# AppleHolic/pytorch_sound

Hardware: AMD Instinct MI355X
Metric: audio-sec/s STFT+mel+fwd/bwd (higher is better)
Workload: dtype bf16; 1 GPU; configs[1]: Conv1d separator (4 x ResBlock1, C=256, on 513-bin magnitude), 22.05 kHz, STFT 1024/256, 80 mel, batch 32 x 2 s per GPU, Adam, bf16 autocast; global_batch=32, parallelism=dp1, model_params=5520386

## Files before the change

pytorch_sound_amd/csrc/psnd_conv.hip:

```cpp
#include "psnd_common.h"
#include "psnd_conv_pair.h"
#include <stdlib.h>
#include <string.h>
#include <algorithm>
#include <atomic>

namespace {

typedef __attribute__((ext_vector_type(8))) short bf16x8;
typedef __attribute__((ext_vector_type(16))) float f32x16;
typedef unsigned short bf16_t;

__device__ __forceinline__ float bf2f(bf16_t v) { return __builtin_bit_cast(float, (unsigned)v << 16); }
__device__ __forceinline__ bf16_t f2bf(float f) {
    unsigned u = __builtin_bit_cast(unsigned, f);
    if ((u & 0x7fffffffu) > 0x7f800000u) return (bf16_t)((u >> 16) | 0x40);
    u += 0x7fffu + ((u >> 16) & 1u);
    return (bf16_t)(u >> 16);
}

typedef __bf16 hwbf16x2 __attribute__((ext_vector_type(2)));
typedef float f32x2_t __attribute__((ext_vector_type(2)));
__device__ __forceinline__ unsigned pack_bf16(float lo, float hi) {
    const f32x2_t v = {lo, hi};
// ... 446 lines not shown
    float l1acc = 0.f;
#pragma unroll
    for (int i = 0; i < 4; ++i) {
        const int j = ty + 8 * i, c = c0 + j, t = t0 + tx;
        if (c < C && t < T) {
            const size_t o = clip + (size_t)c * T + t;
            const float v = MASK ? tile[tx][j] * m[i] : tile[tx][j];
            out[o] = v;
            if (l1) l1acc += fabsf(v - r[i]);
        }
    }
    if (MASK && l1_part) {
        double d = (double)l1acc;
#pragma unroll
        for (int m = 32; m >= 1; m >>= 1) d += __shfl_xor(d, m, 64);
        __shared__ double red[4];
        if ((threadIdx.x & 63) == 0) red[threadIdx.x >> 6] = d;
        __syncthreads();
        if (threadIdx.x == 0)
            l1_part[((size_t)blockIdx.z * gridDim.y + blockIdx.y) * gridDim.x + blockIdx.x] = red[0] + red[1] + red[2] + red[3];
    }
}

constexpr int WKT = 3;
struct WgradParams {
    const bf16_t *G1, *G2, *GM;
    const bf16_t *xa;
    float *gw, *gbias;
    bf16_t *g_out;
    long long R;
    int Ca, Cb, k, off0, dstep, rows_per_split;
    float g2_slope;
    int up_u, up_p, up_Lp, up_HP, up_LpO, up_HPO, up_Cr;
#ifdef PSND_TRACE
    long long *trace;
#endif
};
#ifdef PSND_TRACE
#define PSND_WSTAMP(i_)                                                                                         \
    do {                                                                                                        \
        if ((threadIdx.x & 63) == 0 && p.trace)                                                                 \
            p.trace[(tblk * 4 + (threadIdx.x >> 6)) * 8 + (i_)] = __builtin_amdgcn_s_memtime(); \
    } while (0)
#else
#define PSND_WSTAMP(i_)
#endif

#ifndef PSND_WD
#define PSND_WD 2
#endif
constexpr int WD = PSND_WD;
#ifndef PSND_WGRAD_WAVES
#define PSND_WGRAD_WAVES 2
#endif
constexpr int kWgradLdsBytes = 2 * (1 + WKT) * 64 * RS * (int)sizeof(bf16_t);
__device__ __forceinline__ void conv_wgrad_body_v1(const WgradParams &p, const int bx, const int by, const int bz, bf16_t *sT, const size_t tblk) {
    const int tid = threadIdx.x, wave = tid >> 6, lane = tid & 63;
    const int wm = wave >> 1, wn = wave & 1, li = lane & 31, kg = lane >> 5;
    const int co0 = bx * 64, ci0 = by * 64;
    const int ntg = (p.k + WKT - 1) / WKT;
    const int split = bz / ntg, tgrp = bz - split * ntg;
    const long long rs = (long long)split * p.rows_per_split;
    const long long re = min(rs + p.rows_per_split, p.R);
    const int rr = tid & 31, cg = tid >> 5;
    const bool do_bias = (by == 0) && tgrp == 0;
    const bool comb = p.G2 != nullptr;
// ... 124 lines not shown
                    }
                }
        }
    }
    PSND_WSTAMP(3);
#ifdef PSND_TRACE
    __builtin_amdgcn_s_waitcnt(0);
    PSND_WSTAMP(4);
#endif
    if (do_bias && p.gbias) {
#pragma unroll
        for (int e = 0; e < 8; ++e) {
            float v = bsum[e];
#pragma unroll
            for (int m = 16; m >= 1; m >>= 1) v += __shfl_xor(v, m, 64);
            if (rr == 0 && co0 + 8 * cg + e < p.Cb) p.gbias[(size_t)split * p.Cb + co0 + 8 * cg + e] = v;
        }
    }
}
typedef short v4s_t __attribute__((ext_vector_type(4)));
#ifndef PSND_WGRAD_TR
#define PSND_WGRAD_TR 1
#endif
constexpr int WTP = 96;
constexpr int WXR = 64;
static_assert(2 * (32 + WXR) * WTP * (int)sizeof(bf16_t) <= kWgradLdsBytes, "the transposing-read tiles fit version 1's LDS");
__device__ __forceinline__ bf16x8 tr_frag(const bf16_t *p0) {
    const v4s_t a = __builtin_amdgcn_ds_read_tr16_b64_v4i16((v4s_t __attribute__((address_space(3))) *)(p0));
    const v4s_t b = __builtin_amdgcn_ds_read_tr16_b64_v4i16((v4s_t __attribute__((address_space(3))) *)(p0 + 4 * WTP));
    return __builtin_shufflevector(a, b, 0, 1, 2, 3, 4, 5, 6, 7);
}
constexpr int WXRN = 96;
constexpr int kWgradNarrowLdsBytes = 2 * (32 + WXRN) * WTP * (int)sizeof(bf16_t);
template <bool COMB, bool NARROW = false, int WK = WKT>
__device__ __forceinline__ void conv_wgrad_body(const WgradParams &p, const int bx, const int by, const int bz, bf16_t *sT, const size_t tblk) {
#if !PSND_WGRAD_TR
    conv_wgrad_body_v1(p, bx, by, bz, sT, tblk);
#else
    constexpr int XU = NARROW ? 3 : 2, XR = NARROW ? WXRN : WXR, TPW = NARROW ? 4 * WK : WK;
    const int tid = threadIdx.x, wave = tid >> 6, lane = tid & 63;
    const int wm = NARROW ? 0 : wave >> 1, wn = NARROW ? 0 : wave & 1, li = lane & 31, kg = lane >> 5;
    const int co0 = bx * 64, ci0 = by * 64;
    const int ntg = (p.k + TPW - 1) / TPW;
    const int split = bz / ntg, tgrp = bz - split * ntg;
    const long long rs = (long long)split * p.rows_per_split;
    const long long re = min(rs + p.rows_per_split, p.R);
    const int rr = tid >> 3, cg = tid & 7;
    const bool do_bias = (by == 0) && tgrp == 0;
    constexpr bool comb = COMB;
    const bool gok = co0 + 8 * cg < p.Cb, xok = ci0 + 8 * cg < p.Ca;
    float bsum[8] = {0.f, 0.f, 0.f, 0.f, 0.f, 0.f, 0.f, 0.f};
    PSND_WSTAMP(0);
    constexpr unsigned OOB = 0xffffffffu;
    const int g_bytes = (int)((size_t)p.R * p.Cb * sizeof(bf16_t));
    const int x_bytes = p.up_u > 0 ? (int)((size_t)(p.R / p.up_Lp) * p.up_LpO * p.up_Cr * sizeof(bf16_t)) : (int)((size_t)p.R * p.Ca * sizeof(bf16_t));
    const bool haveG1 = p.G1 != nullptr;
    const __amdgpu_buffer_rsrc_t rG1 = make_uniform_rsrc(haveG1 ? p.G1 : p.G2, g_bytes);
    const __amdgpu_buffer_rsrc_t rG2 = make_uniform_rsrc(comb ? p.G2 : p.G1, g_bytes);
    const __amdgpu_buffer_rsrc_t rGM = make_uniform_rsrc(comb ? p.GM : p.G1, g_bytes);
    const __amdgpu_buffer_rsrc_t rX = make_uniform_rsrc(p.xa, x_bytes);
    auto ld16 = [&](__amdgpu_buffer_rsrc_t r, unsigned off) __attribute__((always_inline)) {
        const auto v = __builtin_amdgcn_raw_buffer_load_b128(r, (int)off, 0, 0);
        return __builtin_bit_cast(uint4, v);
    };
    const int tw0 = tgrp * TPW, ntw = min(TPW, p.k - tw0);
    const int t0 = NARROW ? tw0 + wave * WK : tw0;
    const int nt = max(0, min(WK, p.k - t0));
// ... 35 lines not shown
            vx[s][u] = ld16(rX, ok ? (unsigned)((xo + ci0 + 8 * cg) * sizeof(bf16_t)) : OOB);
        }
    };
    auto stage = [&](auto sc, long long r0, bf16_t *sG, bf16_t *sX) __attribute__((always_inline)) {
        constexpr int s = decltype(sc)::value;
        uint4 g = vg[s];
        if constexpr (COMB) {
            const unsigned *pv = reinterpret_cast<const unsigned *>(&vg[s]), *pg = reinterpret_cast<const unsigned *>(&vg2[s]),
                           *pm = reinterpret_cast<const unsigned *>(&vgm[s]);
            unsigned out[4];
#pragma unroll
            for (int i = 0; i < 4; ++i) {
                const float a0 = bf2f((bf16_t)(pv[i] & 0xffff)), a1 = bf2f((bf16_t)(pv[i] >> 16));
                const float b0 = bf2f((bf16_t)(pg[i] & 0xffff)), b1 = bf2f((bf16_t)(pg[i] >> 16));
                const float m0 = bf2f((bf16_t)(pm[i] & 0xffff)), m1 = bf2f((bf16_t)(pm[i] >> 16));
                out[i] = pack_bf16(a0 + b0 * (m0 > 0.f ? 1.f : p.g2_slope), a1 + b1 * (m1 > 0.f ? 1.f : p.g2_slope));
            }
            g = make_uint4(out[0], out[1], out[2], out[3]);
        }
        if (do_bias) {
            const unsigned *pg4 = reinterpret_cast<const unsigned *>(&g);
#pragma unroll
            for (int e = 0; e < 8; ++e) bsum[e] += bf2f((bf16_t)((pg4[e >> 1] >> (16 * (e & 1))) & 0xffff));
            const long long r = r0 + rr;
            if (p.g_out && r < re && gok) *reinterpret_cast<uint4 *>(p.g_out + (size_t)r * p.Cb + co0 + 8 * cg) = g;
        }
        *reinterpret_cast<uint4 *>(sG + rr * WTP + 8 * cg) = g;
        *reinterpret_cast<uint4 *>(sX + rr * WTP + 8 * cg) = vx[s][0];
        if (rr + 32 < xrows) *reinterpret_cast<uint4 *>(sX + (rr + 32) * WTP + 8 * cg) = vx[s][1];
        if constexpr (NARROW)
            if (rr + 64 < xrows) *reinterpret_cast<uint4 *>(sX + (rr + 64) * WTP + 8 * cg) = vx[s][2];
    };
    const int trow = 8 * kg + ((lane & 15) >> 2), tcol = 16 * ((lane >> 4) & 1) + 4 * (lane & 3);
    const int nchunk = ((int)((re - rs + 31) / 32) + WD - 1) / WD * WD;
    static_for<0, WD>([&](auto sc) __attribute__((always_inline)) { fetch(sc, rs + 32ll * decltype(sc)::value); });
    for (int c = 0; c < nchunk; c += WD) {
        static_for<0, WD>([&](auto sc) __attribute__((always_inline)) {
            constexpr int s = decltype(sc)::value;
            const int ch = c + s;
            bf16_t *sG = sT + (ch & 1) * (32 + XR) * WTP, *sX = sG + 32 * WTP;
            if (ch == 4) PSND_WSTAMP(5);
            stage(sc, rs + 32ll * ch, sG, sX);
            if (ch == 0) PSND_WSTAMP(1);
            if (ch == 4) PSND_WSTAMP(6);
            __syncthreads();
            if (ch == 4) PSND_WSTAMP(7);
            fetch(sc, rs + 32ll * (ch + WD));
            bf16x8 fa[2], fb[2][WK];
#pragma unroll
            for (int kk = 0; kk < 2; ++kk) {
                fa[kk] = tr_frag(sG + (16 * kk + trow) * WTP + wm * 32 + tcol);
#pragma unroll
                for (int j = 0; j < WK; ++j) fb[kk][j] = tr_frag(sX + (16 * kk + trow + toff[j]) * WTP + wn * 32 + tcol);
            }
#pragma unroll
            for (int kk = 0; kk < 2; ++kk)
#pragma unroll
                for (int j = 0; j < WK; ++j) acc[j] = __builtin_amdgcn_mfma_f32_32x32x16_bf16(fa[kk], fb[kk][j], acc[j], 0, 0, 0);
        });
    }
    __syncthreads();
    PSND_WSTAMP(2);
    if constexpr (NARROW) {
        constexpr int EPN = 36;
        float *sE = reinterpret_cast<float *>(sT);
        static_assert(4 * 32 * EPN * 4 <= kWgradNarrowLdsBytes, "four 32 x 32 blocks fit the chunk buffers");
        const bool vec = (p.Ca % 4 == 0);
#pragma unroll
        for (int j = 0; j < WK; ++j) {
            if (j > 0) __syncthreads();
#pragma unroll
            for (int rg = 0; rg < 16; ++rg) sE[(wave * 32 + (rg & 3) + 8 * (rg >> 2) + 4 * kg) * EPN + li] = acc[j][rg];
            __syncthreads();
#pragma unroll
            for (int u = 0; u < 4; ++u) {
                const int idx = tid + 256 * u, w = idx >> 8, row = (idx >> 3) & 31, c4 = 4 * (idx & 7);
                const int tap = tw0 + w * WK + j;
                const int co = co0 + row, ci = ci0 + c4;
                if (tap >= p.k || co >= p.Cb || ci >= p.Ca) continue;
                float *dst = p.gw + (((size_t)split * p.k + tap) * p.Cb) * p.Ca;
                const f32x4 v = *reinterpret_cast<const f32x4 *>(sE + (w * 32 + row) * EPN + c4);
                if (vec && ci + 3 < p.Ca) {
                    *reinterpret_cast<f32x4 *>(dst + (size_t)co * p.Ca + ci) = v;
                } else {
                    const float e[4] = {v.x, v.y, v.z, v.w};
                    for (int q = 0; q < 4 && ci + q < p.Ca; ++q) dst[(size_t)co * p.Ca + ci + q] = e[q];
                }
            }
        }
    } else {
        constexpr int EP = 68;
        float *sE = reinterpret_cast<float *>(sT);
        static_assert(64 * EP * 4 <= kWgradLdsBytes, "one tap's slab tile fits the chunk buffers");
// ... 11 lines not shown
                    const int idx = tid + 256 * u, row = idx >> 4, c4 = 4 * (idx & 15);
                    const int co = co0 + row, ci = ci0 + c4;
                    if (co >= p.Cb || ci >= p.Ca) continue;
                    const f32x4 v = *reinterpret_cast<const f32x4 *>(sE + row * EP + c4);
                    if (vec && ci + 3 < p.Ca) {
                        *reinterpret_cast<f32x4 *>(dst + (size_t)co * p.Ca + ci) = v;
                    } else {
                        const float e[4] = {v.x, v.y, v.z, v.w};
                        for (int q = 0; q < 4 && ci + q < p.Ca; ++q) dst[(size_t)co * p.Ca + ci + q] = e[q];
                    }
                }
            }
    }
    __syncthreads();
    PSND_WSTAMP(3);
#ifdef PSND_TRACE
    __builtin_amdgcn_s_waitcnt(0);
    PSND_WSTAMP(4);
#endif
    if (do_bias && p.gbias) {
        float *sb = reinterpret_cast<float *>(sT);
#pragma unroll
        for (int e = 0; e < 8; ++e) {
            float v = bsum[e];
#pragma unroll
            for (int m = 32; m >= 8; m >>= 1) v += __shfl_xor(v, m, 64);
            if ((lane >> 3) == 0) sb[wave * 64 + 8 * cg + e] = v;
        }
        __syncthreads();
        if (tid < 64 && co0 + tid < p.Cb) p.gbias[(size_t)split * p.Cb + co0 + tid] = (sb[tid] + sb[64 + tid]) + (sb[128 + tid] + sb[192 + tid]);
    }
#endif
}
__global__ __launch_bounds__(256, PSND_WGRAD_WAVES) void conv_wgrad_kernel(WgradParams p) {
    extern __shared__ __attribute__((aligned(16))) bf16_t smem_dyn[];
    if (p.G2) conv_wgrad_body<true>(p, blockIdx.x, blockIdx.y, blockIdx.z, smem_dyn, ((size_t)blockIdx.z * gridDim.y + blockIdx.y) * gridDim.x + blockIdx.x);
    else conv_wgrad_body<false>(p, blockIdx.x, blockIdx.y, blockIdx.z, smem_dyn, ((size_t)blockIdx.z * gridDim.y + blockIdx.y) * gridDim.x + blockIdx.x);
}

constexpr int pair_wk(int KT, int HMX) { return HMX != 25 ? WKT : (KT >= 9 ? 6 : (KT >= 5 ? 4 : WKT)); }
template <int KT, int D, int NBUF, bool COMBINE, int MT, int HMX = 25, int KCT = 32, int WNC = 2, bool WN = false>
__global__ __launch_bounds__(256, (D == 1 ? 3 : PSND_CONV_OCC)) void conv_bwd_pair_kernel(ConvParams pc, WgradParams pw, int nw, int wgx, int wgy, int cgx) {
    extern __shared__ __attribute__((aligned(16))) bf16_t smem_dyn[];
    const int b = blockIdx.x;
    if (b < nw) {
        const int bx = b % wgx, r = b / wgx;
        conv_wgrad_body<COMBINE, WN, ((WN || D == 1) ? WKT : pair_wk(KT, HMX))>(pw, bx, r % wgy, r / wgy, smem_dyn, 0);
    } else {
        const int c = b - nw;
        conv_cl_body<KT, D, COMBINE, NBUF, MT, HMX, false, KCT, WNC>(pc, c % cgx, c / cgx, smem_dyn, 0);
    }
}


#ifndef PSND_PAIRBWD_MR
#define PSND_PAIRBWD_MR 1
#endif
#ifndef PSND_PAIRBWD_RU
#define PSND_PAIRBWD_RU 6
#endif
__global__ __launch_bounds__(256, 2) void conv_pair_bwd_kernel(pairk::PairParams pp, WgradParams wa, WgradParams wb_, int nwa, int nwb, int wgx,
                                                               int wgy) {
    extern __shared__ __attribute__((aligned(16))) bf16_t smem_dyn[];
    const int b = blockIdx.x;
    if (b < nwa) {
        const int bx = b % wgx, r = b / wgx;
        conv_wgrad_body<false>(wa, bx, r % wgy, r / wgy, smem_dyn, 0);
    } else if (b < nwa + nwb) {
        const int c = b - nwa, bx = c % wgx, r = c / wgx;
        conv_wgrad_body<false>(wb_, bx, r % wgy, r / wgy, smem_dyn, 0);
    } else {
        pairk::conv_pair_body<256, PSND_PAIRBWD_MR, true, 4, PSND_PAIRBWD_RU>(pp, b - nwa - nwb, smem_dyn);
    }
}

constexpr int WGRAD_MULTI_MAX = 32;
struct WgradMultiArgs {
    WgradParams base;
    int n, linear, ci_fastest;
    struct {
        const bf16_t *g, *xa;
        float *gw, *gb;
        int off0, dstep, Ca, Cb, k, rps, wgx, wgy, splits, tiles, lab0;
    } c[WGRAD_MULTI_MAX];
};
__global__ __launch_bounds__(256, 2) void conv_wgrad_multi_kernel(WgradMultiArgs a) {
    extern __shared__ __attribute__((aligned(16))) bf16_t smem_dyn[];
    const bool lin = a.linear != 0;
    const int label = lin ? 0 : (int)(blockIdx.x & 7), sh = lin ? 0 : 3;
    int t = (int)blockIdx.x >> sh, c = 0, split = 0;
    for (; c < a.n; ++c) {
        const int first = lin ? 0 : (label - a.c[c].lab0) & 7, S = a.c[c].splits, T = a.c[c].tiles;
        const int nb = first < S ? (((S - first - 1) >> sh) + 1) * T : 0;
        if (t < nb) {
            split = first + ((t / T) << sh), t = t % T;
            break;
        }
        t -= nb;
    }
    if (c == a.n) return;
    WgradParams w = a.base;
    w.G1 = a.c[c].g, w.xa = a.c[c].xa, w.gw = a.c[c].gw, w.gbias = a.c[c].gb, w.off0 = a.c[c].off0, w.dstep = a.c[c].dstep;
    w.Ca = a.c[c].Ca, w.Cb = a.c[c].Cb, w.k = a.c[c].k, w.rows_per_split = a.c[c].rps;
    const int wgx = a.c[c].wgx, wgy = a.c[c].wgy, txy = t % (wgx * wgy), tgrp = t / (wgx * wgy);
    const int bx = a.ci_fastest ? txy / wgy : txy % wgx, by = a.ci_fastest ? txy % wgy : txy / wgx;
    conv_wgrad_body<false>(w, bx, by, split * (a.c[c].tiles / (wgx * wgy)) + tgrp, smem_dyn, 0);
}

__global__ __launch_bounds__(256) void conv_prep_kernel(const float *v, const float *g, const float *bias, int Cout, int Cin, int k,
                                                        int Cb, int Ca, bf16_t *wf, bf16_t *wb, float *bp) {
    __shared__ float red[4];
    const int co = blockIdx.x, n = Cin * k;
    const float *vr = v + (size_t)co * n;
    float ss = 0.f;
    for (int i = threadIdx.x; i < n; i += 256) ss = __builtin_fmaf(vr[i], vr[i], ss);
    for (int m = 32; m >= 1; m >>= 1) ss += __shfl_xor(ss, m, 64);
    if ((threadIdx.x & 63) == 0) red[threadIdx.x >> 6] = ss;
    __syncthreads();
    const float scale = g[co] / __builtin_sqrtf(red[0] + red[1] + red[2] + red[3]);
    for (int i = threadIdx.x; i < n; i += 256) {
        const int ci = i / k, j = i - ci * k;
        const bf16_t w = f2bf(vr[i] * scale);
        wf[pack_index(k, j, co, ci, Cb, Ca)] = w;
        wb[pack_index(k, j, ci, co, Ca, Cb)] = w;
    }
    if (threadIdx.x == 0) bp[co] = bias ? bias[co] : 0.f;
}

struct PrepDesc {
    const float *v, *g, *bias;
    bf16_t *wf, *wb;
    float *bp;
    int Cout, Cin, k, Cb, Ca, blk0;
};
constexpr int PREP_ROWS = 8;
__global__ __launch_bounds__(256) void conv_prep_multi_kernel(const PrepDesc *descs, int n, int which) {
    extern __shared__ __attribute__((aligned(16))) bf16_t s_prep[];
    int lo = 0, hi = n - 1;
    while (lo < hi) {
// ... 557 lines not shown
        }                                                                                                             \
        hipLaunchKernelGGL(kern, grid, dim3(256), lds, st, p);                                                        \
    } while (0)
    if (p.up_role != 0) {
        if (k > 3 || hm > 25) PSND_FAIL(PSND_E_UNSUPPORTED, "%s: transposed-conv mode is a 2-tap convolution", what);
        if (!combine) PSND_CONV_LAUNCH(3, 8, false, 25, true);
        else PSND_CONV_LAUNCH(3, 4, true, 25, true);
    } else if (hm > 25 && !combine) PSND_CONV_LAUNCH(7, 3, false, 40, false);
    else if (hm > 25) PSND_CONV_LAUNCH(7, 3, true, 40, false);
    else if (k <= 3 && !combine) PSND_CONV_LAUNCH(3, 8, false, 25, false);
    else if (k <= 3) PSND_CONV_LAUNCH(3, 4, true, 25, false);
    else if (k <= 7 && !combine) PSND_CONV_LAUNCH(7, 3, false, 25, false);
    else if (k <= 7) PSND_CONV_LAUNCH(7, 3, true, 25, false);
    else if (k <= 11 && !combine) PSND_CONV_LAUNCH(11, 2, false, 25, false);
    else if (k <= 11) PSND_CONV_LAUNCH(11, 2, true, 25, false);
    else if (!combine) PSND_CONV_LAUNCH(16, 2, false, 25, false);
    else PSND_CONV_LAUNCH(16, 2, true, 25, false);
#undef PSND_CONV_LAUNCH
    hipError_t e_ = hipGetLastError();
    if (e_ != hipSuccess) PSND_FAIL(PSND_E_HIP, "%s: %s", what, hipGetErrorString(e_));
    g_conv_stats[mt == 2 ? 1 : 0]++;
    return PSND_OK;
}

static void conv_params_plain(ConvParams &p) {
    p.up_role = 0, p.up_u = 0, p.up_p = 0, p.up_LpO = 0, p.up_HPO = 0, p.up_LO = 0, p.up_Cr = 0;
    p.res_is_a_eff = 0;
#ifdef PSND_TRACE
    p.trace = nullptr;
#endif
}
static void wgrad_params_plain(WgradParams &p) {
    p.up_u = 0, p.up_p = 0, p.up_Lp = 0, p.up_HP = 0, p.up_LpO = 0, p.up_HPO = 0, p.up_Cr = 0;
#ifdef PSND_TRACE
    p.trace = nullptr;
#endif
}

extern "C" int psnd_conv1d_cl(const void *A, const void *A2, const void *AM, float a2_slope, const void *W, const float *bias,
                              const void *res, const void *mask_src, int64_t N, int Lp, int L, int HP, int Ca, int Cb, int k,
                              int off0, int dstep, float act_slope, float mask_slope, void *out_raw, void *out_act,
                              void *a_eff_out, void *stream) {
    if ((!A && !A2) || !W || (!out_raw && !out_act) || (A2 && !AM)) PSND_FAIL(PSND_E_ARG, "conv1d_cl: null pointer");
    if (a_eff_out && !A2) PSND_FAIL(PSND_E_ARG, "conv1d_cl: a_eff_out needs the combined operand (A2, AM)");
    if (Ca % 32 != 0 || Cb % 8 != 0) PSND_FAIL(PSND_E_SHAPE, "conv1d_cl: Ca=%d must be a multiple of 32, Cb=%d of 8", Ca, Cb);
    if (Cb % 32 != 0) PSND_FAIL(PSND_E_SHAPE, "conv1d_cl: Cb=%d must be a multiple of 32 (fragment-ordered weight pack)", Cb);
    if (k < 1 || k > 16 || N < 0 || Lp < L + 2 * HP || L <= 0) PSND_FAIL(PSND_E_SHAPE, "conv1d_cl: k=%d N=%lld Lp=%d L=%d HP=%d", k, (long long)N, Lp, L, HP);
    int hm = 0;
    for (int j = 0; j < k; ++j) {
        const int o = off0 + j * dstep;
        hm = (o < 0 ? -o : o) > hm ? (o < 0 ? -o : o) : hm;
    }
    if (hm > HP) PSND_FAIL(PSND_E_SHAPE, "conv1d_cl: tap reach %d exceeds the halo HP=%d", hm, HP);
    if (N == 0) return PSND_OK;
    if ((size_t)N * Lp * (Ca > Cb ? Ca : Cb) * 2 >= ((size_t)1 << 32) || (size_t)k * Cb * Ca * 2 >= ((size_t)1 << 32))
        PSND_FAIL(PSND_E_SHAPE, "conv1d_cl: operand larger than 4 GB (32-bit buffer offsets)");
    ConvParams p;
    conv_params_plain(p);
    p.A = static_cast<const bf16_t *>(A), p.A2 = static_cast<const bf16_t *>(A2), p.AM = static_cast<const bf16_t *>(AM);
    p.a2_slope = a2_slope;
    p.W = static_cast<const bf16_t *>(W), p.bias = bias;
    p.res = static_cast<const bf16_t *>(res), p.mask_src = static_cast<const bf16_t *>(mask_src);
    p.out_raw = static_cast<bf16_t *>(out_raw), p.out_act = static_cast<bf16_t *>(out_act);
    p.a_eff_out = static_cast<bf16_t *>(a_eff_out);
    p.R = N * (int64_t)Lp, p.Lp = Lp, p.L = L, p.HP = HP, p.Ca = Ca, p.Cb = Cb, p.k = k, p.off0 = off0, p.dstep = dstep, p.hm = hm;
    p.act_slope = act_slope, p.mask_slope = mask_slope;
// ... 122 lines not shown
    if (rps_out) *rps_out = rps;
    return (int)splits;
}

extern "C" int psnd_conv1d_cl_wgrad_splits(int64_t N, int Lp, int Ca, int Cb, int k) {
    if (N <= 0 || Lp <= 0 || Ca <= 0 || Cb <= 0 || k <= 0) return 0;
    return wgrad_splits(N * (int64_t)Lp, Ca, Cb, k, nullptr);
}

extern "C" int psnd_conv1d_cl_wgrad(const void *G1, const void *G2, const void *GM, float g2_slope, const void *xa, int64_t N,
                                    int Lp, int Ca, int Cb, int k, int off0, int dstep, float *gw_part, float *gbias_part,
                                    void *g_out, void *stream) {
    if ((!G1 && !G2) || (G2 && !GM) || !xa || !gw_part) PSND_FAIL(PSND_E_ARG, "conv1d_cl_wgrad: null pointer");
    if (Ca % 8 != 0 || Cb % 8 != 0 || k < 1 || k > 16 || N < 0) PSND_FAIL(PSND_E_SHAPE, "conv1d_cl_wgrad: Ca=%d Cb=%d k=%d", Ca, Cb, k);
    if ((k < WKT ? k - 1 : WKT - 1) * (dstep < 0 ? -dstep : dstep) > WXR - 32)
        PSND_FAIL(PSND_E_UNSUPPORTED, "conv1d_cl_wgrad: dilation %d: a tap group spans more than %d rows", dstep, WXR - 32);
    if (N == 0) return PSND_OK;
    if ((size_t)N * Lp * (Ca > Cb ? Ca : Cb) * 2 >= ((size_t)1 << 32)) PSND_FAIL(PSND_E_SHAPE, "conv1d_cl_wgrad: operand larger than 4 GB");
    WgradParams p;
    wgrad_params_plain(p);
    p.G1 = static_cast<const bf16_t *>(G1), p.G2 = static_cast<const bf16_t *>(G2), p.GM = static_cast<const bf16_t *>(GM);
    p.xa = static_cast<const bf16_t *>(xa), p.gw = gw_part, p.gbias = gbias_part, p.g_out = static_cast<bf16_t *>(g_out);
    p.R = N * (int64_t)Lp, p.Ca = Ca, p.Cb = Cb, p.k = k, p.off0 = off0, p.dstep = dstep, p.g2_slope = g2_slope;
    const int tx = (Cb + 63) / 64, ty = (Ca + 63) / 64;
    int64_t rps;
    const int splits = wgrad_splits(p.R, Ca, Cb, k, &rps);
    p.rows_per_split = (int)rps;
#ifdef PSND_TRACE
    {
        const char *tp = PSND_ENV("PSND_TRACE_PTR");
        p.trace = tp ? reinterpret_cast<long long *>(strtoull(tp, nullptr, 0)) : nullptr;
    }
#endif
    hipLaunchKernelGGL(conv_wgrad_kernel, dim3(tx, ty, (unsigned)(splits * ((k + WKT - 1) / WKT))), dim3(256), kWgradLdsBytes,
                       static_cast<hipStream_t>(stream), p);
    PSND_CHECK_LAUNCH("conv1d_cl_wgrad");
    return PSND_OK;
}

static int wgrad_multi_splits(int64_t R, int Ca, int Cb, int k, int n, int64_t *rps_out) {
    const int tiles = ((Ca + 63) / 64) * ((Cb + 63) / 64) * ((k + WKT - 1) / WKT);
    int64_t target = 768;
    if (const char *e = PSND_ENV("PSND_WGRAD_MULTI_BLOCKS")) target = psnd_env_int(e, target, 1, 65535);
    int64_t splits = target / ((int64_t)tiles * (n > 0 ? n : 1));
    if (splits < 1) splits = 1;
    int64_t rps = (R + splits - 1) / splits;
    rps = (rps + 31) / 32 * 32;
    if (rps < 64) rps = 64;
    splits = (R + rps - 1) / rps;
    if (rps_out) *rps_out = rps;
    return (int)splits;
}

extern "C" int psnd_conv1d_cl_wgrad_multi_splits(int64_t N, int Lp, int Ca, int Cb, int k, int n_convs) {
    if (N <= 0 || Lp <= 0 || Ca <= 0 || Cb <= 0 || k <= 0 || n_convs <= 0) return 0;
    return wgrad_multi_splits(N * (int64_t)Lp, Ca, Cb, k, n_convs, nullptr);
}

extern "C" int psnd_conv1d_cl_wgrad_multi(const psnd_wgrad_desc *d, int n, int64_t N, int Lp, void *stream) {
    if (!d || n < 0) PSND_FAIL(PSND_E_ARG, "conv1d_cl_wgrad_multi: null pointer");
    if (n == 0 || N == 0) return PSND_OK;
    if (n > WGRAD_MULTI_MAX) PSND_FAIL(PSND_E_UNSUPPORTED, "conv1d_cl_wgrad_multi: %d convs (at most %d per launch)", n, WGRAD_MULTI_MAX);
    if (N < 0 || Lp <= 0) PSND_FAIL(PSND_E_SHAPE, "conv1d_cl_wgrad_multi: N=%lld Lp=%d", (long long)N, Lp);
    const int64_t R = N * (int64_t)Lp;
    WgradMultiArgs a;
    memset(&a, 0, sizeof(a));
    wgrad_params_plain(a.base);
// ... 16 lines not shown
        a.c[i].gw = d[i].gw_part, a.c[i].gb = d[i].gbias_part, a.c[i].off0 = d[i].off0, a.c[i].dstep = d[i].dstep;
        a.c[i].Ca = Ca, a.c[i].Cb = Cb, a.c[i].k = k, a.c[i].rps = (int)rps;
        a.c[i].wgx = (Cb + 63) / 64, a.c[i].wgy = (Ca + 63) / 64, a.c[i].splits = splits;
        a.c[i].tiles = a.c[i].wgx * a.c[i].wgy * ((k + WKT - 1) / WKT);
    }
    if (const char *e = PSND_ENV("PSND_WGRAD_MULTI_MAP")) a.linear = !strcmp(e, "linear");
    if (const char *e = PSND_ENV("PSND_WGRAD_MULTI_ORDER")) a.ci_fastest = !strcmp(e, "ci");
    int64_t load[8] = {0, 0, 0, 0, 0, 0, 0, 0}, total = 0;
    int order[WGRAD_MULTI_MAX];
    for (int i = 0; i < n; ++i) order[i] = i;
    std::stable_sort(order, order + n, [&](int x, int y) { return a.c[x].tiles > a.c[y].tiles; });
    for (int oi = 0; oi < n; ++oi) {
        const int i = order[oi], S = a.c[i].splits;
        int best = 0;
        int64_t best_max = -1, best_sq = 0;
        for (int o = 0; o < 8 && !a.linear; ++o) {
            int64_t mx = 0, sq = 0;
            for (int l = 0; l < 8; ++l) {
                const int first = (l - o) & 7;
                const int64_t v = load[l] + (first < S ? (int64_t)((S - first - 1) / 8 + 1) * a.c[i].tiles : 0);
                mx = v > mx ? v : mx, sq += v * v;
            }
            if (best_max < 0 || mx < best_max || (mx == best_max && sq < best_sq)) best = o, best_max = mx, best_sq = sq;
        }
        a.c[i].lab0 = best;
        for (int l = 0; l < 8; ++l) {
            const int first = (l - best) & 7;
            if (first < S) load[l] += (int64_t)((S - first - 1) / 8 + 1) * a.c[i].tiles;
        }
        total += (int64_t)S * a.c[i].tiles;
    }
    if (!a.linear) total = 8 * *std::max_element(load, load + 8);
    if (total > 0x7fffffff) PSND_FAIL(PSND_E_SHAPE, "conv1d_cl_wgrad_multi: %lld workgroups", (long long)total);
    hipLaunchKernelGGL(conv_wgrad_multi_kernel, dim3((unsigned)total), dim3(256), kWgradLdsBytes, static_cast<hipStream_t>(stream), a);
    PSND_CHECK_LAUNCH("conv1d_cl_wgrad_multi");
    return PSND_OK;
}

static int pair_bwd_splits(int64_t R, int C, int k, int64_t *rps_out) {
    const int tiles = ((C + 63) / 64) * ((C + 63) / 64) * ((k + WKT - 1) / WKT);
    int64_t target = 112;
    if (const char *e = PSND_ENV("PSND_PAIRBWD_BLOCKS")) target = psnd_env_int(e, target, 1, 65535);
    int64_t splits = target / tiles;
    if (splits < 1) splits = 1;
    int64_t rps = (R + splits - 1) / splits;
    rps = (rps + 31) / 32 * 32;
    if (rps < 64) rps = 64;
    splits = (R + rps - 1) / rps;
    if (rps_out) *rps_out = rps;
    return (int)splits;
}

extern "C" int psnd_conv1d_cl_pair_bwd_supported(int C, int k, int pad2, int dil2, int pad1, int dil1) {
    return C == 256 && k == 3 && psnd_conv1d_cl_pair_supported(C, k, pad2, -dil2, pad1, -dil1) && 32 - 2 * pairk::reach3(pad1, -dil1) >= 16 ? 1 : 0;
}

extern "C" int psnd_conv1d_cl_pair_bwd_splits(int64_t N, int Lp, int C, int k) {
    if (N <= 0 || Lp <= 0 || C <= 0 || k <= 0) return 0;
    return pair_bwd_splits(N * (int64_t)Lp, C, k, nullptr);
}

extern "C" int psnd_conv1d_cl_pair_bwd(const void *G, const void *wb2, const void *M1, float m1_slope, void *g_mid, const void *wb1, const void *M2,
                                       float m2_slope, const void *res, int64_t N, int Lp, int L, int HP, int C, int k, int pad2, int dil2,
                                       int pad1, int dil1, void *gx, const void *xa_a, float *gw_a, float *gb_a, const void *G_b,
                                       const void *xa_b, int off_b, int dstep_b, float *gw_b, float *gb_b, void *stream) {
    const bool have_pair = G != nullptr;
    const bool have_b = G_b != nullptr;
    if (!have_pair && !have_b) return PSND_OK;
    if (N <= 0 || Lp <= 0 || L <= 0 || HP < 0 || Lp < L + HP) PSND_FAIL(PSND_E_SHAPE, "conv1d_cl_pair_bwd: N=%lld Lp=%d L=%d HP=%d", (long long)N, Lp, L, HP);
    if (C != 256 || k != 3) PSND_FAIL(PSND_E_UNSUPPORTED, "conv1d_cl_pair_bwd: C=%d k=%d (256 channels, 3 taps)", C, k);
    if ((size_t)N * Lp * C * 2 >= ((size_t)1 << 31)) PSND_FAIL(PSND_E_SHAPE, "conv1d_cl_pair_bwd: operand larger than 2 GB");
    if (have_pair && (!wb2 || !wb1 || !M1 || !g_mid || !gx || !xa_a || !gw_a)) PSND_FAIL(PSND_E_ARG, "conv1d_cl_pair_bwd: null pointer");
    if (have_pair && !psnd_conv1d_cl_pair_bwd_supported(C, k, pad2, dil2, pad1, dil1))
        PSND_FAIL(PSND_E_UNSUPPORTED, "conv1d_cl_pair_bwd: taps (%d,%d) (%d,%d)", pad2, dil2, pad1, dil1);
    if (have_b && (!xa_b || !gw_b)) PSND_FAIL(PSND_E_ARG, "conv1d_cl_pair_bwd: null pointer (second weight gradient)");
    const int64_t R = N * (int64_t)Lp;
    int64_t rps;
    const int splits = pair_bwd_splits(R, C, k, &rps);
    const int wgx = (C + 63) / 64, wgy = (C + 63) / 64, wgz = splits * ((k + WKT - 1) / WKT);
    auto fill = [&](WgradParams &w, const void *g, const void *xa, int off0, int dstep, float *gw, float *gb) {
        wgrad_params_plain(w);
        w.G1 = static_cast<const bf16_t *>(g), w.G2 = nullptr, w.GM = nullptr;
        w.xa = static_cast<const bf16_t *>(xa), w.gw = gw, w.gbias = gb, w.g_out = nullptr;
        w.R = R, w.Ca = C, w.Cb = C, w.k = k, w.off0 = off0, w.dstep = dstep, w.g2_slope = 1.f, w.rows_per_split = (int)rps;
    };
    WgradParams wa, wb_;
    fill(wa, G, xa_a, -pad2, dil2, gw_a, gb_a);
    fill(wb_, G_b, xa_b, off_b, dstep_b, gw_b, gb_b);
    pairk::PairParams pp;
    memset(&pp, 0, sizeof(pp));
    int tiles = 0;
    size_t lds = kWgradLdsBytes;
    if (have_pair) {
        pp.A = static_cast<const pairk::bf16_t *>(G), pp.W1 = static_cast<const pairk::bf16_t *>(wb2), pp.W2 = static_cast<const pairk::bf16_t *>(wb1);
        pp.bias1 = nullptr, pp.bias2 = nullptr;
        pp.M1 = static_cast<const pairk::bf16_t *>(M1), pp.M2 = static_cast<const pairk::bf16_t *>(M2), pp.res = static_cast<const pairk::bf16_t *>(res);
        pp.mid_out = static_cast<pairk::bf16_t *>(g_mid), pp.out_raw = static_cast<pairk::bf16_t *>(gx), pp.out_act = nullptr;
        pp.R = R, pp.Lp = Lp, pp.L = L, pp.HP = HP;
        pp.off1 = pad2, pp.dstep1 = -dil2, pp.h1 = pairk::reach3(pad2, -dil2);
        pp.off2 = pad1, pp.dstep2 = -dil1, pp.h2 = pairk::reach3(pad1, -dil1);
        pp.m1_slope = m1_slope, pp.m2_slope = m2_slope, pp.act1_slope = 1.f, pp.act2_slope = 1.f, pp.trace = nullptr;
        const int MRW = 32 * PSND_PAIRBWD_MR, TS = MRW - 2 * pp.h2;
        tiles = (int)((R + TS - 1) / TS);
        const size_t lp = (size_t)(MRW + 2 * pp.h1 + MRW + 2 * pp.h2) * (C + 8) * 2, lo = (size_t)MRW * (C + 8) * 4;
        if (lds < lp) lds = lp;
        if (lds < lo) lds = lo;
    }
    const int nwa = have_pair ? wgx * wgy * wgz : 0, nwb = have_b ? wgx * wgy * wgz : 0;
    hipLaunchKernelGGL(conv_pair_bwd_kernel, dim3((unsigned)(nwa + nwb + tiles)), dim3(256), lds, static_cast<hipStream_t>(stream), pp, wa, wb_, nwa,
                       nwb, wgx, wgy);
    PSND_CHECK_LAUNCH("conv1d_cl_pair_bwd");
    if (have_pair) g_conv_pair_stats[2]++;
    g_conv_pair_stats[3].store(splits);
    return PSND_OK;
}

extern "C" int psnd_conv1d_cl_bwd(const void *G1, const void *G2, const void *GM, float g2_slope, const void *wb, const void *xa,
                                  int64_t N, int Lp, int L, int HP, int Ca, int Cb, int k, int pad, int dil, void *gx, void *g_out,
                                  const void *gx_mask, float gx_mask_slope, const void *gx_res, float *gw_part, float *gbias_part,
                                  void *stream) {
    static const bool no_pair = PSND_ENV("PSND_NO_BWD_PAIR") != nullptr;
    if (gw_part && (k < WKT ? k - 1 : WKT - 1) * (dil < 0 ? -dil : dil) > WXR - 32)
        PSND_FAIL(PSND_E_UNSUPPORTED, "conv1d_cl_bwd: dilation %d: a tap group spans more than %d rows", dil, WXR - 32);
    int hm = 0;
    for (int j = 0; j < k; ++j) {
// ... 22 lines not shown
    pc.out_raw = static_cast<bf16_t *>(gx), pc.out_act = nullptr, pc.a_eff_out = static_cast<bf16_t *>(g_out);
    if (gx_res && gx_res == g_out) {
        if (Ca != Cb) PSND_FAIL(PSND_E_SHAPE, "conv1d_cl_bwd: gx_res == g_out needs Ca == Cb");
        pc.res = nullptr, pc.res_is_a_eff = 1;
    }
    pc.R = N * (int64_t)Lp, pc.Lp = Lp, pc.L = L, pc.HP = HP, pc.Ca = Cb, pc.Cb = Ca, pc.k = k, pc.off0 = pad, pc.dstep = -dil, pc.hm = hm;
    pc.act_slope = 1.f, pc.mask_slope = gx_mask_slope;
    WgradParams pw;
    wgrad_params_plain(pw);
    pw.G1 = pc.A, pw.G2 = pc.A2, pw.GM = pc.AM;
    pw.xa = static_cast<const bf16_t *>(xa), pw.gw = gw_part, pw.gbias = gbias_part, pw.g_out = nullptr;
    pw.R = pc.R, pw.Ca = Ca, pw.Cb = Cb, pw.k = k, pw.off0 = -pad, pw.dstep = dil, pw.g2_slope = g2_slope;
    int64_t rps;
    const int splits = wgrad_splits(pw.R, Ca, Cb, k, &rps);
    pw.rows_per_split = (int)rps;
    const char *pe = PSND_ENV("PSND_PAIR_MT");
    const int pair_mt = pe ? atoi(pe) : 0;
    const bool can3 = !G2 && hm <= 25 && Ca > 32;
    const int mt = (pair_mt == 1 || pair_mt == 2 || (pair_mt == 3 && can3)) ? pair_mt : ((can3 && conv_row_tiles(pc.R, Ca, true) == 3) ? 3 : 2);
    const bool narrow = Ca <= 32 && mt == 2 && hm <= 25 && !G2 && (pc.R + 63) / 64 >= 1024 && !PSND_ENV("PSND_CONV_NO_NARROW");
    const int bm = narrow ? 256 : 64 * mt, bn = narrow ? 32 : BN;
    const int cgx = (int)((pc.R + bm - 1) / bm), cgy = (Ca + bn - 1) / bn;
    const bool wn = Ca <= 32 && Cb <= 32 && (pc.R + 63) / 64 >= 1024 && hm <= 25 && gw_part &&
                    ((k < 4 * WKT ? k : 4 * WKT) - 1) * (dil < 0 ? -dil : dil) <= WXRN - 32 && !PSND_ENV("PSND_CONV_NO_NARROW");
    const bool narrow1 = narrow && Cb <= 32;
    const int wk = wn ? 4 * WKT : (narrow1 ? WKT : pair_wk(k <= 3 ? 3 : (k <= 7 ? 7 : (k <= 11 ? 11 : 16)), hm > 25 ? 40 : 25));
    if (gw_part && !wn && ((k < wk ? k : wk) - 1) * (dil < 0 ? -dil : dil) > WXR - 32)
        PSND_FAIL(PSND_E_UNSUPPORTED, "conv1d_cl_bwd: dilation %d: a group of %d taps spans more than %d rows", dil, wk, WXR - 32);
    const int wgx = (Cb + 63) / 64, wgy = (Ca + 63) / 64, wgz = splits * ((k + wk - 1) / wk);
    const int nw = wgx * wgy * wgz;
    const int kct = 32;
    size_t lds = 2 * sizeof(bf16_t) * (kct + 8) * (size_t)(bm + 2 * hm);
    if (lds < sizeof(float) * bm * (bn + 8)) lds = sizeof(float) * bm * (bn + 8);
    if (lds < (size_t)kWgradLdsBytes) lds = kWgradLdsBytes;
    if (wn && lds < (size_t)kWgradNarrowLdsBytes) lds = kWgradNarrowLdsBytes;
    hipStream_t st = static_cast<hipStream_t>(stream);
#define PSND_PAIR_LAUNCH(KT_, D_, C_, H_)                                                                              \
    do {                                                                                                              \
        auto kern = mt == 2 ? conv_bwd_pair_kernel<KT_, (C_ ? 2 : (D_ > 4 ? 4 : D_)), 2, C_, 2, H_> : conv_bwd_pair_kernel<KT_, D_, 2, C_, 1, H_>;   \
        if constexpr (H_ == 25 && !C_) {                                                                              \
            if (mt == 3) kern = conv_bwd_pair_kernel<KT_, (D_ > 4 ? 4 : D_), 2, false, 3, H_>;                        \
        }                                                                                                             \
        if constexpr (H_ == 25) {                                                                                     \
            if (wn && mt == 2) kern = conv_bwd_pair_kernel<KT_, (C_ ? 2 : (D_ > 4 ? 4 : D_)), 2, C_, 2, H_, 32, 2, true>;   \
        }                                                                                                             \
        if constexpr (H_ == 25 && !C_) {                                                                              \
            if (narrow1 && wn) kern = conv_bwd_pair_kernel<KT_, 1, 2, false, 2, H_, 32, 1, true>;    \
            else if (narrow1) kern = conv_bwd_pair_kernel<KT_, 1, 2, false, 2, H_, 32, 1>;                            \
            else if (narrow) kern = conv_bwd_pair_kernel<KT_, (D_ > 4 ? 4 : D_), 2, false, 2, H_, 32, 1>;             \
        }                                                                                                             \
        if (lds > 64 * 1024) {                                                                                        \
            hipError_t e = hipFuncSetAttribute(reinterpret_cast<const void *>(kern),                                  \
                                               hipFuncAttributeMaxDynamicSharedMemorySize, (int)lds);                 \
            if (e != hipSuccess) PSND_FAIL(PSND_E_HIP, "conv1d_cl_bwd: set LDS size: %s", hipGetErrorString(e));      \
        }                                                                                                             \
        hipLaunchKernelGGL(kern, dim3((unsigned)(nw + cgx * cgy)), dim3(256), lds, st, pc, pw, nw, wgx, wgy, cgx);    \
    } while (0)
    if (hm > 25 && !G2) PSND_PAIR_LAUNCH(7, 3, false, 40);
    else if (hm > 25) PSND_PAIR_LAUNCH(7, 3, true, 40);
    else if (k <= 3 && !G2) PSND_PAIR_LAUNCH(3, 8, false, 25);
    else if (k <= 3) PSND_PAIR_LAUNCH(3, 4, true, 25);
    else if (k <= 7 && !G2) PSND_PAIR_LAUNCH(7, 3, false, 25);
    else if (k <= 7) PSND_PAIR_LAUNCH(7, 3, true, 25);
    else if (k <= 11 && !G2) PSND_PAIR_LAUNCH(11, 2, false, 25);
    else if (k <= 11) PSND_PAIR_LAUNCH(11, 2, true, 25);
    else if (!G2) PSND_PAIR_LAUNCH(16, 2, false, 25);
    else PSND_PAIR_LAUNCH(16, 2, true, 25);
// ... 368 lines not shown
extern "C" int psnd_convtr1d_cl_bwd(const void *g_raw, const void *g_act, const void *act, float act_slope, const void *wb, const void *xa,
                                    int64_t N, int Lp, int L, int HP, int Cip, int Cr, int stride, int padding, int LpO, int HPO, void *gx,
                                    void *g_eff, float *gw_part, void *stream) {
    if ((!g_raw && !g_act) || (g_act && !act) || !wb || !xa || (!gx && !gw_part)) PSND_FAIL(PSND_E_ARG, "convtr1d_cl_bwd: null pointer");
    if (g_act && !g_eff) PSND_FAIL(PSND_E_ARG, "convtr1d_cl_bwd: g_eff (the combined gradient, N x LpO x Cr) is needed when g_act is given");
    int rc = convtr_check("convtr1d_cl_bwd", N, Lp, L, HP, Cip, Cr, stride, padding, LpO, HPO);
    if (rc != PSND_OK) return rc;
    if (N == 0) return PSND_OK;
    hipStream_t st = static_cast<hipStream_t>(stream);
    ConvParams p;
    conv_params_plain(p);
    p.A = static_cast<const bf16_t *>(g_raw), p.A2 = static_cast<const bf16_t *>(g_act), p.AM = static_cast<const bf16_t *>(act);
    p.a2_slope = act_slope;
    p.W = static_cast<const bf16_t *>(wb), p.bias = nullptr, p.res = nullptr, p.mask_src = nullptr;
    p.out_raw = static_cast<bf16_t *>(gx), p.out_act = nullptr, p.a_eff_out = g_act ? static_cast<bf16_t *>(g_eff) : nullptr;
    p.R = N * (int64_t)Lp, p.Lp = Lp, p.L = L, p.HP = HP, p.Ca = stride * Cr, p.Cb = Cip, p.k = 2, p.off0 = 0, p.dstep = 1, p.hm = 1;
    p.act_slope = 1.f, p.mask_slope = 1.f;
    p.up_role = 2, p.up_u = stride, p.up_p = padding, p.up_LpO = LpO, p.up_HPO = HPO, p.up_LO = L * stride, p.up_Cr = Cr;
    if (gx) {
        rc = conv_launch(p, st, "convtr1d_cl_bwd(data)");
        if (rc != PSND_OK) return rc;
    }
    if (!gw_part) return PSND_OK;
    WgradParams w;
    wgrad_params_plain(w);
    w.G1 = static_cast<const bf16_t *>(xa), w.G2 = nullptr, w.GM = nullptr;
    w.xa = g_act ? static_cast<const bf16_t *>(g_eff) : static_cast<const bf16_t *>(g_raw);
    w.gw = gw_part, w.gbias = nullptr, w.g_out = nullptr;
    w.R = p.R, w.Ca = stride * Cr, w.Cb = Cip, w.k = 2, w.off0 = 0, w.dstep = 1, w.g2_slope = 1.f;
    w.up_u = stride, w.up_p = padding, w.up_Lp = Lp, w.up_HP = HP, w.up_LpO = LpO, w.up_HPO = HPO, w.up_Cr = Cr;
    int64_t rps;
    const int splits = wgrad_splits(w.R, w.Ca, w.Cb, 2, &rps);
    w.rows_per_split = (int)rps;
    hipLaunchKernelGGL(conv_wgrad_kernel, dim3((w.Cb + 63) / 64, (w.Ca + 63) / 64, (unsigned)splits), dim3(256), kWgradLdsBytes, st, w);
    PSND_CHECK_LAUNCH("convtr1d_cl_bwd(wgrad)");
    return PSND_OK;
}

extern "C" int psnd_convtr1d_wnorm_bwd(const float *gw_part, int splits, const float *v, const float *g, int Cin, int Cout, int K, int stride,
                                       int Cr, int Cip, float *gv, float *gg, void *stream) {
    if (!gw_part || !v || !g || !gv || !gg || splits < 1) PSND_FAIL(PSND_E_ARG, "convtr1d_wnorm_bwd: null pointer / splits");
    if (K != 2 * stride) PSND_FAIL(PSND_E_SHAPE, "convtr1d_wnorm_bwd: K=%d stride=%d", K, stride);
    const size_t lds = sizeof(float) * ((size_t)Cout * K + 1024);
    if (lds > 64 * 1024) PSND_FAIL(PSND_E_SHAPE, "convtr1d_wnorm_bwd: Cout*K=%d too large", Cout * K);
    hipLaunchKernelGGL(convtr_finish_kernel, dim3(Cin), dim3(splits > 16 ? 1024 : 256), lds, static_cast<hipStream_t>(stream), gw_part, splits,
                       v, g, Cin, Cout, K, stride, Cr, Cip, gv, gg);
    PSND_CHECK_LAUNCH("convtr1d_wnorm_bwd");
    return PSND_OK;
}


static __global__ __launch_bounds__(256) void cl_colsum_partial_kernel(const bf16_t *g, long long rows, int C, int splits, float *part, int Lp, int lo,
                                                                        int hi) {
    __shared__ float red[256 * 8];
    const int cols8 = C >> 3;
    const int rpp = 256 / cols8;
    const int tid = threadIdx.x, cg = tid % cols8, rr = tid / cols8;
    const long long r0 = rows * blockIdx.x / splits, r1 = rows * (blockIdx.x + 1) / splits;
    float acc[8] = {0.f, 0.f, 0.f, 0.f, 0.f, 0.f, 0.f, 0.f};
    if (rr < rpp) {
        int l = Lp > 0 ? (int)((r0 + rr) % Lp) : 0;
        for (long long r = r0 + rr; r < r1; r += rpp) {
            const bool in = Lp <= 0 || (l >= lo && l < hi);
            if (Lp > 0) {
                l += rpp;
                while (l >= Lp) l -= Lp;
            }
// ... 109 lines not shown
```

Before: 106,500 audio-s/s.

## Feed multi-layer wgrad through an LDS-DMA ring buffer with buffer_load lds

Adds a weight-gradient path that uses buffer_load ... lds to copy gradient and activation tiles straight from global memory into a WNS-deep swizzled LDS ring. Each chunk waits on vmcnt and a single barrier, so the loads skip the register-staging round trip and more chunks can be in flight. It is enabled by default only in the multi-conv wgrad kernel, which now launches with the larger LDS size. The cost is more LDS per workgroup, which can lower occupancy, plus hand-written inline asm with M0 and vmcnt bookkeeping.

```diff
diff --git a/pytorch_sound_amd/csrc/psnd_conv.hip b/pytorch_sound_amd/csrc/psnd_conv.hip
--- a/pytorch_sound_amd/csrc/psnd_conv.hip
+++ b/pytorch_sound_amd/csrc/psnd_conv.hip
@@ -502,6 +502,7 @@
     int Ca, Cb, k, off0, dstep, rows_per_split;
     float g2_slope;
     int up_u, up_p, up_Lp, up_HP, up_LpO, up_HPO, up_Cr;
+    int stage;
 #ifdef PSND_TRACE
     long long *trace;
 #endif
@@ -692,7 +693,27 @@
 }
 constexpr int WXRN = 96;
 constexpr int kWgradNarrowLdsBytes = 2 * (32 + WXRN) * WTP * (int)sizeof(bf16_t);
-template <bool COMB, bool NARROW = false, int WK = WKT>
+#ifndef PSND_WNS
+#define PSND_WNS 4
+#endif
+constexpr int WNS = PSND_WNS;
+constexpr int WDP = 64;
+constexpr int kWgradDmaSlot = (32 + WXR) * WDP;
+constexpr int kWgradDmaLdsBytes = WNS * kWgradDmaSlot * (int)sizeof(bf16_t);
+static_assert(WNS >= 3 && 3 * (WNS - 2) <= 63 && kWgradDmaLdsBytes < 64 * 1024, "vmcnt is a 6-bit counter; M0 carries a 16-bit LDS offset");
+constexpr int kWgradMultiLdsBytes = kWgradDmaLdsBytes > kWgradLdsBytes ? kWgradDmaLdsBytes : kWgradLdsBytes;
+#ifdef PSND_LAB
+constexpr int kWgradLaunchLdsBytes = kWgradMultiLdsBytes;
+#else
+constexpr int kWgradLaunchLdsBytes = kWgradLdsBytes;
+#endif
+__device__ __forceinline__ int wdma_f(int r) { return 4 * ((r >> 1) & 1); }
+__device__ __forceinline__ bf16x8 tr_frag_dma(const bf16_t *p0) {
+    const v4s_t a = __builtin_amdgcn_ds_read_tr16_b64_v4i16((v4s_t __attribute__((address_space(3))) *)(p0));
+    const v4s_t b = __builtin_amdgcn_ds_read_tr16_b64_v4i16((v4s_t __attribute__((address_space(3))) *)(p0 + 4 * WDP));
+    return __builtin_shufflevector(a, b, 0, 1, 2, 3, 4, 5, 6, 7);
+}
+template <bool COMB, bool NARROW = false, int WK = WKT, bool DMA = false>
 __device__ __forceinline__ void conv_wgrad_body(const WgradParams &p, const int bx, const int by, const int bz, bf16_t *sT, const size_t tblk) {
 #if !PSND_WGRAD_TR
     conv_wgrad_body_v1(p, bx, by, bz, sT, tblk);
@@ -794,6 +815,85 @@
             if (rr + 64 < xrows) *reinterpret_cast<uint4 *>(sX + (rr + 64) * WTP + 8 * cg) = vx[s][2];
     };
     const int trow = 8 * kg + ((lane & 15) >> 2), tcol = 16 * ((lane >> 4) & 1) + 4 * (lane & 3);
+    if constexpr (DMA) {
+        static_assert(!COMB && !NARROW && WK == WKT, "the LDS-DMA ring feeds the plain body only");
+        typedef __attribute__((address_space(3))) char *lds_ptr;
+        const unsigned ring = __builtin_amdgcn_readfirstlane((unsigned)(size_t)((lds_ptr)sT));
+        const unsigned wbase = ring + 1024u * __builtin_amdgcn_readfirstlane((unsigned)wave);
+        auto dma_rsrc = [](const void *ptr, unsigned bytes) __attribute__((always_inline)) {
+            const unsigned long long a = reinterpret_cast<unsigned long long>(ptr);
+            u32x4 d;
+            d.x = __builtin_amdgcn_readfirstlane((unsigned)a);
+            d.y = __builtin_amdgcn_readfirstlane((unsigned)(a >> 32)) & 0xffffu;
+            d.z = __builtin_amdgcn_readfirstlane(bytes);
+            d.w = 0x00020000u;
+            return d;
+        };
+        const u32x4 dG = dma_rsrc(p.G1, (unsigned)g_bytes), dX = dma_rsrc(p.xa, (unsigned)x_bytes);
+        const int cs = cg ^ wdma_f(rr);
+        const bool gokd = co0 + 8 * cs < p.Cb, xokd = ci0 + 8 * cs < p.Ca;
+        auto issue = [&](int ch, unsigned slot) __attribute__((always_inline)) {
+            const long long r0 = rs + 32ll * ch, r = r0 + rr;
+            const unsigned og = (r < re && gokd) ? (unsigned)(((size_t)r * p.Cb + co0 + 8 * cs) * sizeof(bf16_t)) : OOB;
+            unsigned ox[2];
+#pragma unroll
+            for (int u = 0; u < 2; ++u) {
+                const int xi = rr + 32 * u;
+                const long long rx = r0 + lo + xi;
+                const bool ok = xi < xrows && rx >= 0 && rx < p.R && xokd;
+                ox[u] = ok ? (unsigned)(((size_t)rx * p.Ca + ci0 + 8 * cs) * sizeof(bf16_t)) : OOB;
+            }
+            const unsigned d0 = wbase + slot * (unsigned)(kWgradDmaSlot * sizeof(bf16_t)), d1 = d0 + 32u * WDP * sizeof(bf16_t),
+                           d2 = d1 + 32u * WDP * sizeof(bf16_t);
+            asm volatile("s_nop 4\n\t"
+                         "s_mov_b32 m0, %0\n\ts_nop 0\n\tbuffer_load_dwordx4 %3, %6, 0 offen lds\n\t"
+                         "s_mov_b32 m0, %1\n\ts_nop 0\n\tbuffer_load_dwordx4 %4, %7, 0 offen lds\n\t"
+                         "s_mov_b32 m0, %2\n\ts_nop 0\n\tbuffer_load_dwordx4 %5, %7, 0 offen lds"
+                         :: "s"(d0), "s"(d1), "s"(d2), "v"(og), "v"(ox[0]), "v"(ox[1]), "s"(dG), "s"(dX) : "memory");
+        };
+        const int ra = trow * WDP + ((wm * 32 + tcol) ^ (8 * wdma_f(trow)));
+        int rb[WK];
+#pragma unroll
+        for (int j = 0; j < WK; ++j) rb[j] = (32 + trow + toff[j]) * WDP + ((wn * 32 + tcol) ^ (8 * wdma_f(trow + toff[j])));
+        const int bo = rr * WDP + 8 * cs;
+        const int nch = (int)((re - rs + 31) / 32);
+        for (int c = 0; c < WNS - 1; ++c) issue(c, (unsigned)c);
+        auto run = [&](auto bias_c) __attribute__((always_inline)) {
+            constexpr bool BIAS = decltype(bias_c)::value;
+            unsigned slot = 0;
+            for (int ch = 0; ch < nch; ++ch) {
+                if (ch == 4) PSND_WSTAMP(5);
+                asm volatile("s_waitcnt vmcnt(%0)\n\ts_waitcnt lgkmcnt(0)" :: "n"(3 * (WNS - 2)) : "memory");
+                if (ch == 0) PSND_WSTAMP(1);
+                if (ch == 4) PSND_WSTAMP(6);
+                __builtin_amdgcn_s_barrier();
+                if (ch == 4) PSND_WSTAMP(7);
+                issue(ch + WNS - 1, slot == 0 ? WNS - 1 : slot - 1);
+                const bf16_t *sS = sT + slot * kWgradDmaSlot;
+                bf16x8 fa[2], fb[2][WK];
+#pragma unroll
+                for (int kk = 0; kk < 2; ++kk) {
+                    fa[kk] = tr_frag_dma(sS + 16 * kk * WDP + ra);
+#pragma unroll
+                    for (int j = 0; j < WK; ++j) fb[kk][j] = tr_frag_dma(sS + 16 * kk * WDP + rb[j]);
+                }
+                if constexpr (BIAS) {
+                    const uint4 g = *reinterpret_cast<const uint4 *>(sS + bo);
+                    const unsigned *pg4 = reinterpret_cast<const unsigned *>(&g);
+#pragma unroll
+                    for (int e = 0; e < 8; ++e) bsum[e] += bf2f((bf16_t)((pg4[e >> 1] >> (16 * (e & 1))) & 0xffff));
+                }
+#pragma unroll
+                for (int kk = 0; kk < 2; ++kk)
+#pragma unroll
+                    for (int j = 0; j < WK; ++j) acc[j] = __builtin_amdgcn_mfma_f32_32x32x16_bf16(fa[kk], fb[kk][j], acc[j], 0, 0, 0);
+                slot = slot + 1 == WNS ? 0 : slot + 1;
+            }
+        };
+        if (do_bias) run(std::true_type{});
+        else run(std::false_type{});
+        asm volatile("s_waitcnt vmcnt(0)" ::: "memory");
+    } else {
     const int nchunk = ((int)((re - rs + 31) / 32) + WD - 1) / WD * WD;
     static_for<0, WD>([&](auto sc) __attribute__((always_inline)) { fetch(sc, rs + 32ll * decltype(sc)::value); });
     for (int c = 0; c < nchunk; c += WD) {
@@ -821,6 +921,7 @@
                 for (int j = 0; j < WK; ++j) acc[j] = __builtin_amdgcn_mfma_f32_32x32x16_bf16(fa[kk], fb[kk][j], acc[j], 0, 0, 0);
         });
     }
+    }
     __syncthreads();
     PSND_WSTAMP(2);
     if constexpr (NARROW) {
@@ -898,10 +999,22 @@
     }
 #endif
 }
+template <bool DMA>
+__device__ __forceinline__ void conv_wgrad_plain(const WgradParams &p, const int bx, const int by, const int bz, bf16_t *sT, const size_t tblk) {
+#ifdef PSND_LAB
+    if (p.stage == 0 ? DMA : p.stage == 2) conv_wgrad_body<false, false, WKT, true>(p, bx, by, bz, sT, tblk);
+    else conv_wgrad_body<false>(p, bx, by, bz, sT, tblk);
+#else
+    if constexpr (DMA) conv_wgrad_body<false, false, WKT, true>(p, bx, by, bz, sT, tblk);
+    else conv_wgrad_body<false>(p, bx, by, bz, sT, tblk);
+#endif
+}
 __global__ __launch_bounds__(256, PSND_WGRAD_WAVES) void conv_wgrad_kernel(WgradParams p) {
     extern __shared__ __attribute__((aligned(16))) bf16_t smem_dyn[];
-    if (p.G2) conv_wgrad_body<true>(p, blockIdx.x, blockIdx.y, blockIdx.z, smem_dyn, ((size_t)blockIdx.z * gridDim.y + blockIdx.y) * gridDim.x + blockIdx.x);
-    else conv_wgrad_body<false>(p, blockIdx.x, blockIdx.y, blockIdx.z, smem_dyn, ((size_t)blockIdx.z * gridDim.y + blockIdx.y) * gridDim.x + blockIdx.x);
+    const size_t tblk = ((size_t)blockIdx.z * gridDim.y + blockIdx.y) * gridDim.x + blockIdx.x;
+    if (p.G2) conv_wgrad_body<true>(p, blockIdx.x, blockIdx.y, blockIdx.z, smem_dyn, tblk);
+    else if (p.g_out || p.up_u > 0) conv_wgrad_body<false>(p, blockIdx.x, blockIdx.y, blockIdx.z, smem_dyn, tblk);
+    else conv_wgrad_plain<false>(p, blockIdx.x, blockIdx.y, blockIdx.z, smem_dyn, tblk);
 }
 
 constexpr int pair_wk(int KT, int HMX) { return HMX != 25 ? WKT : (KT >= 9 ? 6 : (KT >= 5 ? 4 : WKT)); }
@@ -911,7 +1024,9 @@
     const int b = blockIdx.x;
     if (b < nw) {
         const int bx = b % wgx, r = b / wgx;
-        conv_wgrad_body<COMBINE, WN, ((WN || D == 1) ? WKT : pair_wk(KT, HMX))>(pw, bx, r % wgy, r / wgy, smem_dyn, 0);
+        constexpr int WKP = (WN || D == 1) ? WKT : pair_wk(KT, HMX);
+        if constexpr (!COMBINE && !WN && WKP == WKT) conv_wgrad_plain<false>(pw, bx, r % wgy, r / wgy, smem_dyn, 0);
+        else conv_wgrad_body<COMBINE, WN, WKP>(pw, bx, r % wgy, r / wgy, smem_dyn, 0);
     } else {
         const int c = b - nw;
         conv_cl_body<KT, D, COMBINE, NBUF, MT, HMX, false, KCT, WNC>(pc, c % cgx, c / cgx, smem_dyn, 0);
@@ -931,10 +1046,10 @@
     const int b = blockIdx.x;
     if (b < nwa) {
         const int bx = b % wgx, r = b / wgx;
-        conv_wgrad_body<false>(wa, bx, r % wgy, r / wgy, smem_dyn, 0);
+        conv_wgrad_plain<false>(wa, bx, r % wgy, r / wgy, smem_dyn, 0);
     } else if (b < nwa + nwb) {
         const int c = b - nwa, bx = c % wgx, r = c / wgx;
-        conv_wgrad_body<false>(wb_, bx, r % wgy, r / wgy, smem_dyn, 0);
+        conv_wgrad_plain<false>(wb_, bx, r % wgy, r / wgy, smem_dyn, 0);
     } else {
         pairk::conv_pair_body<256, PSND_PAIRBWD_MR, true, 4, PSND_PAIRBWD_RU>(pp, b - nwa - nwb, smem_dyn);
     }
@@ -970,7 +1085,7 @@
     w.Ca = a.c[c].Ca, w.Cb = a.c[c].Cb, w.k = a.c[c].k, w.rows_per_split = a.c[c].rps;
     const int wgx = a.c[c].wgx, wgy = a.c[c].wgy, txy = t % (wgx * wgy), tgrp = t / (wgx * wgy);
     const int bx = a.ci_fastest ? txy / wgy : txy % wgx, by = a.ci_fastest ? txy % wgy : txy / wgx;
-    conv_wgrad_body<false>(w, bx, by, split * (a.c[c].tiles / (wgx * wgy)) + tgrp, smem_dyn, 0);
+    conv_wgrad_plain<true>(w, bx, by, split * (a.c[c].tiles / (wgx * wgy)) + tgrp, smem_dyn, 0);
 }
 
 __global__ __launch_bounds__(256) void conv_prep_kernel(const float *v, const float *g, const float *bias, int Cout, int Cin, int k,
@@ -1594,6 +1709,8 @@
 }
 static void wgrad_params_plain(WgradParams &p) {
     p.up_u = 0, p.up_p = 0, p.up_Lp = 0, p.up_HP = 0, p.up_LpO = 0, p.up_HPO = 0, p.up_Cr = 0;
+    const char *ws = PSND_ENV("PSND_WGRAD_STAGE");
+    p.stage = !ws ? 0 : (!strcmp(ws, "regs") ? 1 : (!strcmp(ws, "dma") ? 2 : 0));
 #ifdef PSND_TRACE
     p.trace = nullptr;
 #endif
@@ -1782,7 +1899,7 @@
         p.trace = tp ? reinterpret_cast<long long *>(strtoull(tp, nullptr, 0)) : nullptr;
     }
 #endif
-    hipLaunchKernelGGL(conv_wgrad_kernel, dim3(tx, ty, (unsigned)(splits * ((k + WKT - 1) / WKT))), dim3(256), kWgradLdsBytes,
+    hipLaunchKernelGGL(conv_wgrad_kernel, dim3(tx, ty, (unsigned)(splits * ((k + WKT - 1) / WKT))), dim3(256), kWgradLaunchLdsBytes,
                        static_cast<hipStream_t>(stream), p);
     PSND_CHECK_LAUNCH("conv1d_cl_wgrad");
     return PSND_OK;
@@ -1865,7 +1982,7 @@
     }
     if (!a.linear) total = 8 * *std::max_element(load, load + 8);
     if (total > 0x7fffffff) PSND_FAIL(PSND_E_SHAPE, "conv1d_cl_wgrad_multi: %lld workgroups", (long long)total);
-    hipLaunchKernelGGL(conv_wgrad_multi_kernel, dim3((unsigned)total), dim3(256), kWgradLdsBytes, static_cast<hipStream_t>(stream), a);
+    hipLaunchKernelGGL(conv_wgrad_multi_kernel, dim3((unsigned)total), dim3(256), kWgradMultiLdsBytes, static_cast<hipStream_t>(stream), a);
     PSND_CHECK_LAUNCH("conv1d_cl_wgrad_multi");
     return PSND_OK;
 }
@@ -1923,7 +2040,7 @@
     pairk::PairParams pp;
     memset(&pp, 0, sizeof(pp));
     int tiles = 0;
-    size_t lds = kWgradLdsBytes;
+    size_t lds = kWgradLaunchLdsBytes;
     if (have_pair) {
         pp.A = static_cast<const pairk::bf16_t *>(G), pp.W1 = static_cast<const pairk::bf16_t *>(wb2), pp.W2 = static_cast<const pairk::bf16_t *>(wb1);
         pp.bias1 = nullptr, pp.bias2 = nullptr;
@@ -2012,7 +2129,7 @@
     const int kct = 32;
     size_t lds = 2 * sizeof(bf16_t) * (kct + 8) * (size_t)(bm + 2 * hm);
     if (lds < sizeof(float) * bm * (bn + 8)) lds = sizeof(float) * bm * (bn + 8);
-    if (lds < (size_t)kWgradLdsBytes) lds = kWgradLdsBytes;
+    if (lds < (size_t)kWgradLaunchLdsBytes) lds = kWgradLaunchLdsBytes;
     if (wn && lds < (size_t)kWgradNarrowLdsBytes) lds = kWgradNarrowLdsBytes;
     hipStream_t st = static_cast<hipStream_t>(stream);
 #define PSND_PAIR_LAUNCH(KT_, D_, C_, H_)                                                                              \
@@ -2447,7 +2564,7 @@
     int64_t rps;
     const int splits = wgrad_splits(w.R, w.Ca, w.Cb, 2, &rps);
     w.rows_per_split = (int)rps;
-    hipLaunchKernelGGL(conv_wgrad_kernel, dim3((w.Cb + 63) / 64, (w.Ca + 63) / 64, (unsigned)splits), dim3(256), kWgradLdsBytes, st, w);
+    hipLaunchKernelGGL(conv_wgrad_kernel, dim3((w.Cb + 63) / 64, (w.Ca + 63) / 64, (unsigned)splits), dim3(256), kWgradLaunchLdsBytes, st, w);
     PSND_CHECK_LAUNCH("convtr1d_cl_bwd(wgrad)");
     return PSND_OK;
 }
```

Result: faster. 108,200 audio-s/s (median of 6 runs) (+1.5%).
